# DeepGraphLearning/ULTRA

Measured on AMD Instinct MI355X. Metric: triples scored/sec (all-tail ranking) on FB15k237, higher is better.
Workload: dtype f32

## Files before the change

### ultra_amd/csrc/layer0_kernels.hpp

```cpp
#pragma once

#include <hip/hip_runtime.h>

#include <cstdint>

#include "layer0_update.hpp"
#include "rspmm_kernels.hpp"
#include "torch_math.hpp"

namespace ultra {

__global__ void __launch_bounds__(256) nbf_layer0_fill_kernel(const Layer0Params p) {
    __shared__ __attribute__((aligned(16))) float lds_slot[16 * 80];
    const int l16 = threadIdx.x & 15;
    const L0Vec vec = l0_load_vectors(p, l16);
    float c0[4];
#pragma unroll
    for (int e = 0; e < 4; ++e) c0[e] = vec.bias[e];
    l0_finish(c0, p, vec, lds_slot + (threadIdx.x >> 4) * 80, l16);
    const float4 v = make_float4(c0[0], c0[1], c0[2], c0[3]);
    if (p.out_sr == 64 && p.out_so == p.num_node * 64) {
        float4 *o4 = reinterpret_cast<float4 *>(p.out);
        const long long n16 = (long long)p.n_outer * p.num_node * 16;
        for (long long i = (long long)blockIdx.x * blockDim.x + threadIdx.x; i < n16; i += (long long)gridDim.x * blockDim.x) o4[i] = v;
        return;
    }
    const long long total = (long long)p.n_outer * p.num_node;
    const long long g0 = ((long long)blockIdx.x * blockDim.x + threadIdx.x) >> 4, ng = ((long long)gridDim.x * blockDim.x) >> 4;
    for (long long r = g0; r < total; r += ng) {
        const long long b = r / p.num_node, n = r - b * p.num_node;
        *reinterpret_cast<float4 *>(p.out + b * p.out_so + n * p.out_sr + 4 * l16) = v;
    }
}

__global__ void __launch_bounds__(1024) nbf_layer0_rows_kernel(const Layer0Params p) {
    __shared__ __attribute__((aligned(16))) float lds_wt[128 * 64];
    __shared__ __attribute__((aligned(16))) float lds_vec[64 * 80];
    const int outer = blockIdx.y;
    const int l16 = threadIdx.x & 15;
    const int grp = blockIdx.x * (blockDim.x >> 4) + (threadIdx.x >> 4);
    const int ngrp = gridDim.x * (blockDim.x >> 4);
    long long s = p.src[outer];
    s = s < 0 ? 0 : (s >= p.num_node ? p.num_node - 1 : s);
    const int k0 = p.trow_ptr[s], k1 = p.trow_ptr[s + 1];
    if (blockIdx.x > 0 && k0 + (int)blockIdx.x * (int)(blockDim.x >> 4) >= k1) return;
    const L0Vec vec = l0_load_vectors(p, l16);
    float qv[4];
#pragma unroll
    for (int e = 0; e < 4; ++e) qv[e] = p.q ? p.q[(long long)outer * 64 + 4 * l16 + e] : 1.f;
    {
        const int f = threadIdx.x & 63;
#pragma unroll
        for (int kc = 4 * (threadIdx.x >> 6); kc < 128; kc += 4 * (blockDim.x >> 6)) {
            const float4 wv = *reinterpret_cast<const float4 *>(p.weight + f * 128 + kc);
            lds_wt[(kc + 0) * 64 + f] = wv.x;
            lds_wt[(kc + 1) * 64 + f] = wv.y;
            lds_wt[(kc + 2) * 64 + f] = wv.z;
            lds_wt[(kc + 3) * 64 + f] = wv.w;
        }
    }
    __syncthreads();
    const float *relb = reinterpret_cast<const float *>(p.rel.ptr) + outer * p.rel.stride_outer;
    float *outb = p.out + outer * p.out_so;
    float *slot = lds_vec + (threadIdx.x >> 4) * 80;

    const auto update_row = [&](const float (&agg)[4], bool is_src, long long row) {
        float y[4] = {0.f, 0.f, 0.f, 0.f};
        if (is_src) {
            *reinterpret_cast<float4 *>(slot + 4 * l16) = make_float4(qv[0], qv[1], qv[2], qv[3]);
#pragma unroll
            for (int k4 = 0; k4 < 16; ++k4) {
                const float4 x4 = *reinterpret_cast<const float4 *>(slot + 4 * k4);
                const float xs[4] = {x4.x, x4.y, x4.z, x4.w};
#pragma unroll
                for (int e = 0; e < 4; ++e) {
                    const float4 wv = *reinterpret_cast<const float4 *>(lds_wt + (4 * k4 + e) * 64 + 4 * l16);
                    y[0] = __builtin_fmaf(xs[e], wv.x, y[0]);
                    y[1] = __builtin_fmaf(xs[e], wv.y, y[1]);
                    y[2] = __builtin_fmaf(xs[e], wv.z, y[2]);
                    y[3] = __builtin_fmaf(xs[e], wv.w, y[3]);
                }
            }
        }
        *reinterpret_cast<float4 *>(slot + 4 * l16) = make_float4(agg[0], agg[1], agg[2], agg[3]);
#pragma unroll
        for (int k4 = 0; k4 < 16; ++k4) {
            const float4 a4 = *reinterpret_cast<const float4 *>(slot + 4 * k4);
            const float as[4] = {a4.x, a4.y, a4.z, a4.w};
#pragma unroll
            for (int e = 0; e < 4; ++e) {
                const float4 wv = *reinterpret_cast<const float4 *>(lds_wt + (64 + 4 * k4 + e) * 64 + 4 * l16);
                y[0] = __builtin_fmaf(as[e], wv.x, y[0]);
                y[1] = __builtin_fmaf(as[e], wv.y, y[1]);
                y[2] = __builtin_fmaf(as[e], wv.z, y[2]);
                y[3] = __builtin_fmaf(as[e], wv.w, y[3]);
            }
        }
#pragma unroll
        for (int e = 0; e < 4; ++e) y[e] += vec.bias[e];
        l0_finish(y, p, vec, slot, l16);
        if (is_src && (p.flags & L0_RESIDUAL)) {
#pragma unroll
            for (int e = 0; e < 4; ++e) y[e] += qv[e];
        }
        *reinterpret_cast<float4 *>(outb + row * p.out_sr + 4 * l16) = make_float4(y[0], y[1], y[2], y[3]);
    };

    for (int k = k0 + grp; k < k1; k += ngrp) {
        const int last = k1 - 1;
        const int prev = p.tcol[k > k0 ? k - 1 : k0];
        int tc[4];
#pragma unroll
        for (int u = 0; u < 4; ++u) tc[u] = p.tcol[min(k + u, last)];
        const int target = tc[0];
        if (k > k0 && prev == target) continue;
        int kend = k + 1;
        if (kend < k1 && tc[1] == target) ++kend;
        if (kend == k + 2 && kend < k1 && tc[2] == target) ++kend;
        if (kend == k + 3 && kend < k1 && tc[3] == target) ++kend;
        if (kend == k + 4)
            while (kend < k1 && p.tcol[kend] == target) ++kend;
        const bool is_src = target == (int)s;
        const bool use_max = (p.flags & L0_MAX) != 0;
        const float init = (use_max && is_src && !(p.self_loop[s] & 2)) ? -3.402823466e+38f : 0.f;
        float agg[4] = {init, init, init, init};
        for (int kb = k; kb < kend; kb += 4) {
            float4 rv[4];
            float wv[4];
#pragma unroll
            for (int u = 0; u < 4; ++u) {
                const int kk = min(kb + u, kend - 1);
                const int ty = p.ttype[kk];
                rv[u] = *reinterpret_cast<const float4 *>(relb + (long long)ty * p.rel.stride_row + 4 * l16);
                wv[u] = p.w ? p.w[p.tperm[kk]] : 1.f;
            }
#pragma unroll
            for (int u = 0; u < 4; ++u) {
                if (kb + u < kend) {
                    const float r4[4] = {rv[u].x, rv[u].y, rv[u].z, rv[u].w};
#pragma unroll
                    for (int e = 0; e < 4; ++e) {
                        float m = r4[e] * qv[e];
                        if (p.w) m = wv[u] * m;
                        agg[e] = use_max ? fmaxf(agg[e], m) : agg[e] + m;
                    }
                }
            }
        }
        if (is_src) {
#pragma unroll
            for (int e = 0; e < 4; ++e) agg[e] = use_max ? fmaxf(agg[e], qv[e]) : agg[e] + qv[e];
        }
        update_row(agg, is_src, target);
    }
    if (grp == 0 && !(p.self_loop[s] & 1)) {
        float a0[4];
#pragma unroll
        for (int e = 0; e < 4; ++e) a0[e] = ((p.flags & L0_MAX) && (p.self_loop[s] & 2)) ? fmaxf(qv[e], 0.f) : qv[e];
        update_row(a0, true, s);
    }
}

}
```

### ultra_amd/csrc/layer0_update.hpp

```cpp
#pragma once

#include <hip/hip_runtime.h>

#include <cstdint>

#include "rspmm_kernels.hpp"
#include "torch_math.hpp"

namespace ultra {

enum { L0_LN = 1, L0_RELU = 2, L0_RESIDUAL = 4, L0_MAX = 8, L0_ONLY_FILL = 16, L0_SKIP_FILL = 32 };

struct Layer0Params {
    const int32_t *trow_ptr;
    const int32_t *tcol;
    const int32_t *ttype;
    const int32_t *tperm;
    const uint8_t *self_loop;
    const float *w;
    const int64_t *src;
    const float *q;
    MatArg rel;
    const float *weight;
    const float *bias, *ln_w, *ln_b;
    float *out;
    long long out_so, out_sr;
    long long num_node;
    int32_t n_outer;
    float eps;
    int32_t flags;
};

struct L0Vec {
    float bias[4], ln_w[4], ln_b[4];
};

__device__ __forceinline__ L0Vec l0_load_vectors(const Layer0Params &p, int l16) {
    L0Vec v;
#pragma unroll
    for (int e = 0; e < 4; ++e) {
        v.bias[e] = p.bias ? p.bias[4 * l16 + e] : 0.f;
        v.ln_w[e] = (p.flags & L0_LN) ? p.ln_w[4 * l16 + e] : 1.f;
        v.ln_b[e] = (p.flags & L0_LN) ? p.ln_b[4 * l16 + e] : 0.f;
    }
    return v;
}

__device__ __forceinline__ void l0_finish(float (&y)[4], const Layer0Params &p, const L0Vec &vec, float *slot, const int l16) {
    if (p.flags & L0_LN) {
        *reinterpret_cast<float4 *>(slot + 4 * l16) = make_float4(y[0], y[1], y[2], y[3]);
        float xv[8];
#pragma unroll
        for (int j = 0; j < 8; ++j) xv[j] = slot[8 * j + (l16 & 7)];
        const Moments w = welford8(xv);
        if (l16 < 8) {
            slot[64 + 2 * l16] = w.m1;
            slot[64 + 2 * l16 + 1] = w.m2;
        }
        Moments all[8];
#pragma unroll
        for (int i = 0; i < 8; ++i) all[i] = Moments{slot[64 + 2 * i], slot[64 + 2 * i + 1]};
        float mean, rstd;
        merge8(all, p.eps, mean, rstd);
#pragma unroll
        for (int e = 0; e < 4; ++e) y[e] = ln_apply(y[e], mean, rstd, vec.ln_w[e], vec.ln_b[e]);
    }
    if (p.flags & L0_RELU) {
#pragma unroll
        for (int e = 0; e < 4; ++e) y[e] = fmaxf(y[e], 0.f);
    }
}

}
```

### ultra_amd/csrc/rspmm_api.hip

```cpp
#include <hip/hip_runtime.h>

#include <cstdio>
#include <cstring>
#include <functional>
#include <string>
#include <vector>

#include "device_scope.hpp"
#include "layer0_kernels.hpp"
#include "rspmm_bwd_kernels.hpp"
#include "rspmm_kernels.hpp"
#include "rspmm_order_kernels.hpp"
#include "rspmm_rows_kernels.hpp"
#include "rows_bwd_kernels.hpp"

namespace ultra {

#define ULTRA_EXTERN_VARIANT(T_, VEC_, MODE_) \
    template <>                               \
    hipError_t launch_fwd_variant<T_, VEC_, MODE_>(int, int, const FwdParams &, int, int, size_t, hipStream_t);
ULTRA_EXTERN_VARIANT(float, 4, 0)
ULTRA_EXTERN_VARIANT(float, 1, 0)
ULTRA_EXTERN_VARIANT(float, 4, 1)
ULTRA_EXTERN_VARIANT(float, 4, 2)
// ... 596 lines not shown
    const int64_t step = dtype == ULTRA_F32 ? 4 : 2;
    bool vec4 = (row_len % 4 == 0) && mat_vec_ok(out, step);
    if (mul != BIN_RHS) vec4 = vec4 && mat_vec_ok(rel, step);
    if (mul != BIN_LHS) vec4 = vec4 && mat_vec_ok(x, step);
    if (bnd) vec4 = vec4 && mat_vec_ok(bnd, step);
    if (rot) vec4 = vec4 && (row_len % 8 == 0);
    const int VEC = vec4 ? 4 : 1;
    const int SPAN = 16 * VEC;
    const bool rot_far = rot && !(VEC == 4 && row_len == SPAN);

    if ((p->flags & ULTRA_PLAN_TYPE_RUNS) && !(p->flags & ULTRA_PLAN_EXACT_ORDER)) {
        if (!(sum == ULTRA_SUM_ADD && mul == BIN_MUL)) {
            set_error("a ULTRA_PLAN_TYPE_RUNS plan serves add_mul only (distributivity)");
            return ULTRA_ERR_UNSUPPORTED;
        }
        mul = BIN_MUL_TYPED;
    }
    const auto slice_bytes = [&](const ultra_mat *m, int64_t rows) { return (uint64_t)rows * (uint64_t)m->stride_row * esz; };
    if ((mul != BIN_LHS && slice_bytes(x, p->num_in) >= (1ull << 32)) ||
        (mul != BIN_RHS && slice_bytes(rel, p->num_rel) >= (1ull << 32))) {
        set_error("rspmm: an operand slice (rows * stride_row) exceeds 4 GiB; use the batch-major layout");
        return ULTRA_ERR_UNSUPPORTED;
    }
    FwdParams fp = fwd_params(p, mul, w, rel, x, bnd, out, SPAN, (int64_t)esz, call);

    const size_t ring_bytes = p->n_chain > 0 ? (size_t)2 * CHAIN_SLOTS * 64 * esz : 0;
    if ((p->flags & ULTRA_PLAN_EXACT_ORDER) && !rot && VEC == 4 && general_walk() == 0 && p->num_in < (1 << 24) &&
        p->num_rel < (1 << 24) && (mul == BIN_LHS || x->stride_row * (int64_t)esz < (1 << 24)) &&
        (mul == BIN_RHS || rel->stride_row * (int64_t)esz < (1 << 24)) && ring_bytes <= di.lds_optin)
        return forward_order(p, sum, mul, dtype, w, x, bnd, out, stream, call, fp, di, ring_bytes, point_fill);
    if (call.upd) {
        set_error("ultra_rspmm_forward_update: this call is not served by the reference-order kernels");
        return ULTRA_ERR_UNSUPPORTED;
    }
    if (call.w_samples) {
        set_error("ultra_rspmm_forward_masked_samples: this call is not served by the reference-order kernels (row length, "
                  "alignment or tuning)");
        return ULTRA_ERR_UNSUPPORTED;
    }
    if (point_fill) {
        set_error("a point boundary under min / max: this call is not served by the reference-order kernels (row length, "
                  "alignment or tuning); pass the boundary as a tensor");
        return ULTRA_ERR_UNSUPPORTED;
    }
    return forward_walk(p, sum, mul, dtype, w, bnd, out, stream, call, fp, di, VEC, rot_far);
}

static int ensure_backward_plans(ultra_plan *p) {
    if (p->tplan && p->rplan) return ULTRA_OK;
    if ((int64_t)p->h_row.size() != p->num_edge) return invalid("plan was built without its edge list; backward unavailable");
    ultra_plan_opts o;
    std::memset(&o, 0, sizeof(o));
    o.seg_len = p->seg_len;
    o.g_max = p->g_max;
    o.flags = p->flags & ~ULTRA_PLAN_EXACT_ORDER;
    if (!p->tplan) {
        p->tplan = build_plan(p->h_col.data(), p->h_row.data(), p->h_type.data(), p->num_edge, p->num_in, p->num_out,
                              p->num_rel, &o, false);
        p->tplan->pinned = p->pinned;
    }
    if (!p->rplan) {
        p->rplan = build_plan(p->h_type.data(), p->h_col.data(), p->h_row.data(), p->num_edge, p->num_rel, p->num_in,
                              p->num_out, &o, false);
        p->rplan->pinned = p->pinned;
    }
    return ULTRA_OK;
}

template <typename Launch>
static int backward_gather(ultra_plan *p, int dtype, const void *w, const EdgeParams &ep, const ultra_mat *xgrad,
                           const ultra_mat *rgrad, int32_t spans_per_outer, int fix_vec, const char *what, hipStream_t stream,
                           const Launch &launch) {
    const size_t esz = dtype == ULTRA_F32 ? 4 : 8;
    int rc;
    if ((rc = ensure_backward_plans(p))) return rc;
    for (int which = 0; which < 2; ++which) {
        ultra_plan *q = which == 0 ? p->tplan : p->rplan;
        const ultra_mat *dst = which == 0 ? xgrad : rgrad;
        if ((rc = upload_plan(q))) return rc;
        if (q->n_slot > 0 &&
            (rc = ensure_scratch(&q->d.partial, &q->d.partial_bytes, (size_t)q->n_slot * ep.n_outer * ep.row_len * esz, q)))
            return rc;
        GatherBwdParams gp;
        std::memset(&gp, 0, sizeof(gp));
        gp.items = q->d.items;
        gp.n_item = (int32_t)q->items.size();
        gp.col = q->d.col, gp.type = q->d.type, gp.perm = q->d.perm;
        gp.w = w;
        gp.rel = ep.rel, gp.x = ep.x, gp.out = ep.out, gp.og = ep.og;
        gp.grad = dst->ptr, gp.grad_so = dst->stride_outer, gp.grad_sr = dst->stride_row;
        gp.partial = q->d.partial;
        gp.n_outer = ep.n_outer, gp.row_len = ep.row_len;
        gp.spans_per_outer = spans_per_outer;
        gp.n_span = gp.spans_per_outer * gp.n_outer;
        const int grid = 2048;
        gp.smod = std::min<int32_t>(gp.n_span, grid);
        gp.nparts = grid / gp.smod;
        const hipError_t e = launch(which == 1, gp, grid);
        if (e != hipSuccess) return hip_fail(e, what);
        if ((rc = launch_fixup(q, dst, 0, dtype, fix_vec, stream))) return rc;
    }
    return ULTRA_OK;
}

static int backward_impl(ultra_plan *p, int sum, int mul, int dtype, const void *w, const ultra_mat *rel,
                         const ultra_mat *x, const ultra_mat *outm, const ultra_mat *og, void *wgrad,
                         const ultra_mat *rgrad, const ultra_mat *xgrad, hipStream_t stream, const ultra_mat *xbase = nullptr) {
    if (!p) return invalid("plan is NULL");
    if (xbase && (sum != ULTRA_SUM_ADD || !xgrad)) return invalid("input_grad_base is served under sum == add, with an input_grad");
    (void)hipGetLastError();
    if (p->flags & ULTRA_PLAN_DENSE) return invalid("a ULTRA_PLAN_DENSE plan has no backward; use the (row, col) plan");
    if (sum < 0 || sum > 2 || mul < 0 || mul > ULTRA_MUL_ROTATE) return invalid("unknown sum/mul code");
    const bool rot = mul == ULTRA_MUL_ROTATE;
    if (dtype != ULTRA_F32 && dtype != ULTRA_F64) return invalid("dtype must be ULTRA_F32 or ULTRA_F64");
    if (!og || !og->ptr) return invalid("output_grad is NULL");
    const int64_t n_outer = og->n_outer, row_len = og->row_len;
    if (n_outer <= 0 || row_len <= 0) return invalid("output_grad: empty n_outer / row_len");
    if (rot && (row_len & 1)) return invalid("rotate: row_len must be even (a row is real half | imaginary half)");
    int rc;
    if ((rc = check_mat(rel, "relation", p->num_rel, n_outer, row_len))) return rc;
    if ((rc = check_mat(x, "input", p->num_in, n_outer, row_len))) return rc;
    if ((rc = check_mat(outm, "output", p->num_out, n_outer, row_len))) return rc;
    if ((rc = check_mat(og, "output_grad", p->num_out, n_outer, row_len))) return rc;
    if ((rc = check_mat(rgrad, "relation_grad", p->num_rel, n_outer, row_len))) return rc;
    if (!xgrad && sum != ULTRA_SUM_ADD) return invalid("input_grad may be NULL under sum == add only");
    if (xgrad && (rc = check_mat(xgrad, "input_grad", p->num_in, n_outer, row_len))) return rc;
    if (xbase && (rc = check_mat(xbase, "input_grad_base", p->num_in, n_outer, row_len))) return rc;
    if ((rc = upload_plan(p))) return rc;

    const int64_t step = dtype == ULTRA_F32 ? 4 : 2;
    const bool vec4 = (row_len % 4 == 0) && mat_vec_ok(rel, step) && mat_vec_ok(x, step) && mat_vec_ok(outm, step) &&
                      mat_vec_ok(og, step) && mat_vec_ok(rgrad, step) && (!xgrad || mat_vec_ok(xgrad, step));

    EdgeParams ep;
    std::memset(&ep, 0, sizeof(ep));
    ep.erow = p->d.erow;
    ep.col = p->d.col;
    ep.type = p->d.type;
    ep.perm = p->d.perm;
    ep.w = w;
    ep.num_edge = p->num_edge;
    ep.num_out = (int32_t)p->num_out;
    ep.rel = MatArg{rel->ptr, rel->stride_outer, rel->stride_row};
    ep.x = MatArg{x->ptr, x->stride_outer, x->stride_row};
    ep.out = MatArg{outm->ptr, outm->stride_outer, outm->stride_row};
    ep.og = MatArg{og->ptr, og->stride_outer, og->stride_row};
    ep.rgrad = rgrad->ptr;
    ep.rgrad_so = rgrad->stride_outer;
    ep.rgrad_sr = rgrad->stride_row;
    ep.xgrad = xgrad ? xgrad->ptr : nullptr;
    ep.xgrad_so = xgrad ? xgrad->stride_outer : 0;
    ep.xgrad_sr = xgrad ? xgrad->stride_row : 0;
    ep.wgrad = wgrad;
    ep.n_outer = (int32_t)n_outer;
    ep.row_len = (int32_t)row_len;

    if (sum == ULTRA_SUM_ADD) {
        if ((rc = ensure_backward_plans(p))) return rc;
        if (xgrad && (rc = forward_impl(p->tplan, ULTRA_SUM_ADD, rot ? BIN_ROT_CREL : mul == ULTRA_MUL_MUL ? BIN_MUL : BIN_RHS, dtype,
                                        w, rel, og, xbase, xgrad, stream)))
            return rc;
        if ((rc = forward_impl(p->rplan, ULTRA_SUM_ADD, rot ? BIN_ROT_CX : mul == ULTRA_MUL_MUL ? BIN_MUL : BIN_LHS, dtype, w, og, x,
                               nullptr, rgrad, stream)))
            return rc;
        if (!wgrad || p->num_edge <= 0) return ULTRA_OK;
        if (rot) return launch_rot_edge_kernel(dtype, sum, false, ep, stream);
        return launch_edge_kernel(dtype, vec4 ? 4 : 1, sum, mul, false, ep, stream);
    }
    if (rot && p->num_edge > 0) {
        const bool fix4 = (row_len % 4 == 0) && mat_vec_ok(rgrad, step) && mat_vec_ok(xgrad, step);
        const auto launch = [&](bool rel_grad, const GatherBwdParams &gp, int grid) {
            return dtype == ULTRA_F32 ? launch_rot_gather_bwd_t<float>(sum, rel_grad, gp, grid, stream)
                                      : launch_rot_gather_bwd_t<double>(sum, rel_grad, gp, grid, stream);
        };
        if ((rc = backward_gather(p, dtype, w, ep, xgrad, rgrad, (int32_t)((row_len / 2 + 15) / 16), fix4 ? 4 : 1,
                                  "rspmm_rot_minmax_bwd_gather_kernel launch", stream, launch)))
            return rc;
        return wgrad ? launch_rot_edge_kernel(dtype, sum, false, ep, stream) : ULTRA_OK;
    }
    if (vec4 && row_len % 4 == 0 && p->num_edge > 0) {
        const auto launch = [&](bool rel_grad, const GatherBwdParams &gp, int grid) {
            return dtype == ULTRA_F32 ? launch_gather_bwd_t<float>(sum, mul, rel_grad, gp, grid, stream)
                                      : launch_gather_bwd_t<double>(sum, mul, rel_grad, gp, grid, stream);
        };
        if ((rc = backward_gather(p, dtype, w, ep, xgrad, rgrad, (int32_t)((row_len + 63) / 64), 4,
                                  "rspmm_minmax_bwd_gather_kernel launch", stream, launch)))
            return rc;
        return wgrad ? launch_edge_kernel(dtype, 4, sum, mul, false, ep, stream) : ULTRA_OK;
    }
    if ((rc = launch_fill_zero(dtype, rgrad, p->num_rel, stream))) return rc;
    if ((rc = launch_fill_zero(dtype, xgrad, p->num_in, stream))) return rc;
    if (p->num_edge > 0 && !rot) return launch_edge_kernel(dtype, vec4 ? 4 : 1, sum, mul, true, ep, stream);
    return ULTRA_OK;
}

static int forward_onehot_impl(ultra_plan *p, int dtype, const void *w, const ultra_mat *rel, const ultra_mat *x,
                               const int64_t *src_rows, const ultra_mat *bnd, const ultra_mat *out, hipStream_t stream) {
    if (!p) return invalid("plan is NULL");
    (void)hipGetLastError();
    if (dtype != ULTRA_F32 && dtype != ULTRA_F64) return invalid("dtype must be ULTRA_F32 or ULTRA_F64");
    if (!out || !out->ptr || !src_rows) return invalid("output / src_rows is NULL");
    if (p->flags & (ULTRA_PLAN_TYPE_RUNS | ULTRA_PLAN_DENSE)) return invalid("use the (row, col) plan for the one-hot path");
    const int64_t n_outer = out->n_outer, row_len = out->row_len;
    int rc;
    if ((rc = check_mat(out, "output", p->num_out, n_outer, row_len))) return rc;
    if ((rc = check_mat(rel, "relation", p->num_rel, n_outer, row_len))) return rc;
    if ((rc = check_mat(x, "input", p->num_in, n_outer, row_len))) return rc;
    if (bnd && (rc = check_mat(bnd, "boundary", p->num_out, n_outer, row_len))) return rc;
    if (p->num_out != p->num_in) return invalid("one-hot path needs a square graph (source rows are output rows)");
    if ((rc = ensure_backward_plans(p))) return rc;
    if ((rc = upload_plan(p->tplan))) return rc;
    const size_t esz = dtype == ULTRA_F32 ? 4 : 8;
    if (out->stride_row == row_len && (n_outer == 1 || out->stride_outer == out->n_row * row_len) && out->n_row == p->num_out &&
        aligned16(out->ptr) && ((size_t)n_outer * p->num_out * row_len * esz) % 16 == 0) {
        const long long n16 = (long long)((size_t)n_outer * p->num_out * row_len * esz / 16);
        hipLaunchKernelGGL(zero16_kernel, dim3(1024), dim3(256), 0, stream, reinterpret_cast<float4 *>(out->ptr), n16);
        HIP_TRY(hipGetLastError());
    } else if ((rc = launch_fill_zero(dtype, out, p->num_out, stream))) {
        return rc;
    }
    const int64_t step = dtype == ULTRA_F32 ? 4 : 2;
    const bool vec4 = (row_len % 4 == 0) && mat_vec_ok(out, step) && mat_vec_ok(rel, step) && mat_vec_ok(x, step);
    OneHotParams op;
    std::memset(&op, 0, sizeof(op));
    op.trow_ptr = p->tplan->d.row_ptr;
    op.tcol = p->tplan->d.col;
    op.ttype = p->tplan->d.type;
    op.tperm = p->tplan->d.perm;
    op.w = w;
    op.src = src_rows;
    op.rel = MatArg{rel->ptr, rel->stride_outer, rel->stride_row};
    op.x = MatArg{x->ptr, x->stride_outer, x->stride_row};
    if (bnd) op.bnd = MatArg{bnd->ptr, bnd->stride_outer, bnd->stride_row};
    op.out = out->ptr;
    op.out_so = out->stride_outer;
    op.out_sr = out->stride_row;
    op.n_outer = (int32_t)n_outer;
    op.row_len = (int32_t)row_len;
    op.has_bnd = bnd ? 1 : 0;
    const dim3 grid(64, (unsigned)n_outer), block(256);
    if (dtype == ULTRA_F32) {
        if (vec4) hipLaunchKernelGGL((rspmm_onehot_kernel<float, 4>), grid, block, 0, stream, op);
        else hipLaunchKernelGGL((rspmm_onehot_kernel<float, 1>), grid, block, 0, stream, op);
    } else {
        if (vec4) hipLaunchKernelGGL((rspmm_onehot_kernel<double, 4>), grid, block, 0, stream, op);
        else hipLaunchKernelGGL((rspmm_onehot_kernel<double, 1>), grid, block, 0, stream, op);
    }
    HIP_TRY(hipGetLastError());
    return ULTRA_OK;
}

static int layer0_impl(ultra_plan *p, const void *w, const ultra_mat *rel, const int64_t *src_rows, const void *src_vals,
                       const void *weight, const void *bias, const void *ln_w, const void *ln_b, float eps, int flags,
                       const ultra_mat *out, hipStream_t stream) {
    if (!p) return invalid("plan is NULL");
    (void)hipGetLastError();
    const bool only_fill = (flags & L0_ONLY_FILL) != 0;
    if (flags & ~(L0_LN | L0_RELU | L0_RESIDUAL | L0_MAX | L0_ONLY_FILL | L0_SKIP_FILL))
        return invalid("ultra_nbf_layer0: unknown flag bits " + std::to_string(flags & ~(L0_LN | L0_RELU | L0_RESIDUAL | L0_MAX | L0_ONLY_FILL | L0_SKIP_FILL)));
    if (only_fill && (flags & L0_SKIP_FILL)) return invalid("ultra_nbf_layer0: ULTRA_LAYER0_ONLY_FILL excludes ULTRA_LAYER0_SKIP_FILL");
    if (!out || !out->ptr || (!only_fill && (!src_rows || !weight))) return invalid("ultra_nbf_layer0: NULL operand");
    if ((flags & L0_LN) && (!ln_w || !ln_b)) return invalid("ultra_nbf_layer0: LayerNorm needs its weight and bias");
    if (p->flags & (ULTRA_PLAN_TYPE_RUNS | ULTRA_PLAN_DENSE)) return invalid("use the (row, col) plan for the layer-0 path");
    if (out->row_len != 64) {
        set_error("ultra_nbf_layer0: only hidden dim 64 is built (the ULTRA checkpoints' shape)");
        return ULTRA_ERR_UNSUPPORTED;
    }
    const int64_t n_outer = out->n_outer;
    int rc;
    if ((rc = check_mat(out, "output", p->num_out, n_outer, 64))) return rc;
    if (!only_fill && (rc = check_mat(rel, "relation", p->num_rel, n_outer, 64))) return rc;
    if (p->num_out != p->num_in) return invalid("layer-0 path needs a square graph (source rows are output rows)");
    if (!mat_vec_ok(out, 4) || (!only_fill && (!mat_vec_ok(rel, 4) || !aligned16(weight) || (src_vals && !aligned16(src_vals)))))
        return invalid("ultra_nbf_layer0: operands must be 16-byte aligned with strides that are multiples of 4");
    if (n_outer == 0 || p->num_out == 0) return ULTRA_OK;
    Layer0Params lp;
    std::memset(&lp, 0, sizeof(lp));
    if (!only_fill) {
        if ((rc = ensure_backward_plans(p))) return rc;
        if ((rc = upload_plan(p->tplan))) return rc;
        if ((rc = upload_plan(p))) return rc;
        if (!p->d.self_loop) return invalid("plan was built without its edge list; layer-0 path unavailable");
        lp.trow_ptr = p->tplan->d.row_ptr;
        lp.tcol = p->tplan->d.col;
        lp.ttype = p->tplan->d.type;
        lp.tperm = p->tplan->d.perm;
        lp.self_loop = p->d.self_loop;
        lp.rel = MatArg{rel->ptr, rel->stride_outer, rel->stride_row};
    }
    lp.w = static_cast<const float *>(w);
    lp.src = src_rows;
    lp.q = static_cast<const float *>(src_vals);
    lp.weight = static_cast<const float *>(weight);
    lp.bias = static_cast<const float *>(bias);
    lp.ln_w = static_cast<const float *>(ln_w);
    lp.ln_b = static_cast<const float *>(ln_b);
    lp.out = static_cast<float *>(out->ptr);
    lp.out_so = out->stride_outer;
    lp.out_sr = out->stride_row;
    lp.num_node = p->num_out;
    lp.n_outer = (int32_t)n_outer;
    lp.eps = eps;
    lp.flags = flags;
    const long long rows = (long long)n_outer * p->num_out;
    const int fill_blocks = (int)std::min<long long>((rows + 15) / 16, 1024);
    if (!(flags & L0_SKIP_FILL)) {
        hipLaunchKernelGGL(nbf_layer0_fill_kernel, dim3(fill_blocks), dim3(256), 0, stream, lp);
        HIP_TRY(hipGetLastError());
    }
    if (!only_fill) {
        ultra_plan *tp = p->tplan;
        if (tp->max_row_len < 0) {
            int32_t m = 0;
            for (size_t r = 0; r + 1 < tp->row_ptr.size(); ++r) m = std::max(m, tp->row_ptr[r + 1] - tp->row_ptr[r]);
            tp->max_row_len = m;
        }
        const unsigned l0_blocks = (unsigned)std::min(std::max((tp->max_row_len + 63) / 64, 32), 256);
        hipLaunchKernelGGL(nbf_layer0_rows_kernel, dim3(l0_blocks, (unsigned)n_outer), dim3(1024), 0, stream, lp);
        HIP_TRY(hipGetLastError());
    }
    return ULTRA_OK;
}

static int internal_mul(int32_t *mul) {
    if (*mul < 0 || *mul > ULTRA_MUL_ROTATE) return invalid("unknown mul code");
    if (*mul == ULTRA_MUL_ROTATE) *mul = BIN_ROT;
    return ULTRA_OK;
}

static int forward_update(ultra_plan *plan, int sum, int mul, const ultra_mat *relation, const ultra_mat *input,
                          const ultra_mat *point_values, const ultra_mat *aggregate, const void *weight, const void *bias,
                          const void *ln_weight, const void *ln_bias, float eps, int flags, const ultra_mat *output,
                          hipStream_t stream, FwdCall call) {
    if (mul < 0 || mul > 1) return invalid("unknown mul code");
    if ((call.bnd_rows == nullptr) != (point_values == nullptr)) return invalid("ultra_rspmm_forward_update: half a point boundary");
    if (!weight || !output || !output->ptr || !aggregate || !aggregate->ptr || ((flags & CONV_LN) && (!ln_weight || !ln_bias)))
        return invalid("ultra_rspmm_forward_update: NULL operand");
    if (flags & ~(CONV_LN | CONV_RELU | CONV_RESIDUAL | CONV_DBG_NO_MATRIX | CONV_DBG_NO_UPDATE | CONV_DBG_LOSE_ARRIVAL))
        return invalid("ultra_rspmm_forward_update: unknown flag");
    if (!plan) return invalid("plan is NULL");
    if (output->row_len != 64 || output->n_outer != aggregate->n_outer || output->n_row != aggregate->n_row ||
        output->stride_row < 64 || (output->stride_row % 4) != 0 || (output->stride_outer % 4) != 0 ||
        (reinterpret_cast<uintptr_t>(output->ptr) & 15) || output->ptr == aggregate->ptr || (input && output->ptr == input->ptr))
        return invalid("ultra_rspmm_forward_update: output must be a 16-byte aligned (n_outer, num_node, 64) tensor of its own");
    OrderParams::Update u;
    std::memset(&u, 0, sizeof(u));
    u.weight = (const float *)weight, u.bias = (const float *)bias;
    u.ln_w = (const float *)ln_weight, u.ln_b = (const float *)ln_bias;
    u.out = (float *)output->ptr;
    u.out_stride_outer = output->stride_outer, u.out_stride_row = output->stride_row;
    u.eps = eps, u.flags = flags;
    call.upd = &u;
    return forward_impl(plan, sum, mul, ULTRA_F32, nullptr, relation, input, point_values, aggregate, stream, call);
}

static ultra_mat dense2d(const void *ptr, int64_t rows, int64_t dim) {
    ultra_mat m;
    m.ptr = const_cast<void *>(ptr);
    m.n_outer = 1;
    m.stride_outer = 0;
    m.n_row = rows;
    m.stride_row = dim;
    m.row_len = dim;
    return m;
}

static int stateless_plan(ultra_plan **plan, const int64_t *ei_dev, const int64_t *et_dev, int64_t E, int64_t N,
                          int64_t R, hipStream_t stream) {
    *plan = nullptr;
    if (E < 0 || N < 0 || R < 0) return invalid("negative size");
    std::vector<int64_t> ei((size_t)2 * E), et((size_t)E);
    HIP_TRY(hipStreamSynchronize(stream));
    if (E > 0) {
        HIP_TRY(hipMemcpy(ei.data(), ei_dev, sizeof(int64_t) * 2 * E, hipMemcpyDeviceToHost));
        HIP_TRY(hipMemcpy(et.data(), et_dev, sizeof(int64_t) * E, hipMemcpyDeviceToHost));
        int64_t maxc = 0;
        for (int64_t e = 0; e < E; ++e) maxc = std::max(maxc, ei[(size_t)(E + e)]);
        for (int64_t e = 1; e < E; ++e) {
            const int64_t k0 = ei[(size_t)e - 1] * (maxc + 1) + ei[(size_t)(E + e - 1)];
            const int64_t k1 = ei[(size_t)e] * (maxc + 1) + ei[(size_t)(E + e)];
            if (k1 < k0) {
                set_error("Expect sorted `edge_index`");
                return ULTRA_ERR_UNSORTED;
            }
        }
    }
    ultra_plan_opts opts;
    std::memset(&opts, 0, sizeof(opts));
    opts.flags = ULTRA_PLAN_EXACT_ORDER;
    return ultra_plan_create(plan, ei.data(), et.data(), E, N, N, R, &opts);
}

}

using namespace ultra;

extern "C" {

int32_t ultra_device_count(void) {
    int n = 0;
    if (hipGetDeviceCount(&n) != hipSuccess) return 0;
    return n;
}

int32_t ultra_plan_upload(ultra_plan *plan) {
    if (!plan) return invalid("plan is NULL");
    return upload_plan(plan);
}

int32_t ultra_plan_pin(ultra_plan *plan, int32_t delta) {
    if (!plan) return invalid("plan is NULL");
    const auto bump = [&](ultra_plan *q) { q->pinned = std::max<int32_t>(0, q->pinned + delta); };
    bump(plan);
    if (plan->tplan) bump(plan->tplan);
    if (plan->rplan) bump(plan->rplan);
    return ULTRA_OK;
}

int32_t ultra_plan_destroy(ultra_plan *plan) {
    if (!plan) return ULTRA_OK;
    if (plan->tplan) ultra_plan_destroy(plan->tplan);
    if (plan->rplan) ultra_plan_destroy(plan->rplan);
    free_device(plan);
    delete plan;
    return ULTRA_OK;
}

int32_t ultra_rspmm_weight_epoch(int64_t epoch) {
    g_w_epoch = epoch;
    return ULTRA_OK;
}

int32_t ultra_rspmm_forward(ultra_plan *plan, int32_t sum, int32_t mul, int32_t dtype, const void *edge_weight_dev,
                            const ultra_mat *relation, const ultra_mat *input, const ultra_mat *boundary,
                            const ultra_mat *output, void *stream) {
    ULTRA_DEVICE_SCOPE(stream, output ? output->ptr : nullptr);
    WeightEpochScope weight_epoch_scope;
    if (int rc = internal_mul(&mul)) return rc;
    return forward_impl(plan, sum, mul, dtype, edge_weight_dev, relation, input, boundary, output,
                        reinterpret_cast<hipStream_t>(stream));
}

int32_t ultra_rspmm_forward_masked(ultra_plan *plan, int32_t sum, int32_t mul, int32_t dtype, const void *edge_keep_dev,
                                   const ultra_mat *relation, const ultra_mat *input, const ultra_mat *boundary,
                                   const ultra_mat *output, void *stream) {
    ULTRA_DEVICE_SCOPE(stream, output ? output->ptr : nullptr);
    WeightEpochScope weight_epoch_scope;
    if (int rc = internal_mul(&mul)) return rc;
    if (!edge_keep_dev) return invalid("ultra_rspmm_forward_masked: edge_keep is NULL");
    FwdCall call;
    call.keep_mode = 1;
    return forward_impl(plan, sum, mul, dtype, edge_keep_dev, relation, input, boundary, output,
                        reinterpret_cast<hipStream_t>(stream), call);
}

int32_t ultra_rspmm_forward_masked_samples(ultra_plan *plan, int32_t sum, int32_t mul, int32_t dtype, const void *edge_keep_dev,
                                           int64_t keep_stride, const ultra_mat *relation, const ultra_mat *input,
                                           const ultra_mat *boundary, const ultra_mat *output, void *stream) {
    if (!plan) return invalid("plan is NULL");
    if (keep_stride < plan->num_edge) return invalid("ultra_rspmm_forward_masked_samples: keep_stride < num_edge");
    if (!edge_keep_dev) return invalid("ultra_rspmm_forward_masked_samples: edge_keep is NULL");
    if (!output || !output->ptr) return invalid("output is NULL");
    if (output->n_outer == 0) return ULTRA_OK;
    if (keep_stride > INT32_MAX) {
        set_error("ultra_rspmm_forward_masked_samples: keep_stride beyond 2^31 - 1 elements");
        return ULTRA_ERR_UNSUPPORTED;
    }
    ULTRA_DEVICE_SCOPE(stream, output->ptr);
    WeightEpochScope weight_epoch_scope;
    if (int rc = internal_mul(&mul)) return rc;
    FwdCall call;
    call.keep_mode = 1;
    call.w_samples = true;
    call.w_stride_outer = keep_stride;
    return forward_impl(plan, sum, mul, dtype, edge_keep_dev, relation, input, boundary, output,
                        reinterpret_cast<hipStream_t>(stream), call);
}

int32_t ultra_rspmm_forward_point(ultra_plan *plan, int32_t sum, int32_t mul, int32_t dtype, const void *edge_weight_dev,
                                  const ultra_mat *relation, const ultra_mat *input, const int64_t *point_rows_dev,
                                  const ultra_mat *point_values, const ultra_mat *output, void *stream) {
    ULTRA_DEVICE_SCOPE(stream, output ? output->ptr : nullptr);
    WeightEpochScope weight_epoch_scope;
    if (int rc = internal_mul(&mul)) return rc;
    if (!point_rows_dev || !point_values) return invalid("ultra_rspmm_forward_point: NULL point boundary");
    return forward_impl(plan, sum, mul, dtype, edge_weight_dev, relation, input, point_values, output,
                        reinterpret_cast<hipStream_t>(stream), FwdCall{point_rows_dev});
}

int32_t ultra_rspmm_forward_update(ultra_plan *plan, int32_t sum, int32_t mul, const ultra_mat *relation, const ultra_mat *input,
                                   const int64_t *point_rows_dev, const ultra_mat *point_values, const ultra_mat *aggregate,
                                   const void *weight, const void *bias, const void *ln_weight, const void *ln_bias, float eps,
                                   int32_t flags, const ultra_mat *output, void *stream) {
    ULTRA_DEVICE_SCOPE(stream, output ? output->ptr : nullptr);
    return forward_update(plan, sum, mul, relation, input, point_values, aggregate, weight, bias, ln_weight, ln_bias, eps, flags,
                          output, reinterpret_cast<hipStream_t>(stream), FwdCall{point_rows_dev});
}

int32_t ultra_rspmm_forward_onehot(ultra_plan *plan, int32_t dtype, const void *edge_weight_dev,
                                   const ultra_mat *relation, const ultra_mat *input, const int64_t *src_rows_dev,
                                   const ultra_mat *boundary, const ultra_mat *output, void *stream) {
    ULTRA_DEVICE_SCOPE(stream, output ? output->ptr : nullptr);
    return forward_onehot_impl(plan, dtype, edge_weight_dev, relation, input, src_rows_dev, boundary, output,
                               reinterpret_cast<hipStream_t>(stream));
}

int32_t ultra_nbf_layer0(ultra_plan *plan, const void *edge_weight_dev, const ultra_mat *relation, const int64_t *src_rows_dev,
                         const void *src_values_dev, const void *weight, const void *bias, const void *ln_weight,
                         const void *ln_bias, float eps, int32_t flags, const ultra_mat *output, void *stream) {
    ULTRA_DEVICE_SCOPE(stream, output ? output->ptr : nullptr);
    return layer0_impl(plan, edge_weight_dev, relation, src_rows_dev, src_values_dev, weight, bias, ln_weight, ln_bias, eps,
                       flags, output, reinterpret_cast<hipStream_t>(stream));
}

int32_t ultra_nbf_dense_layer(ultra_plan *plan, const ultra_mat *relation, const ultra_mat *input, const ultra_mat *boundary,
                              const int64_t *point_rows_dev, const void *weight, const void *bias, const void *ln_weight,
                              const void *ln_bias, float eps, int32_t flags, const ultra_mat *output, void *stream) {
    ULTRA_DEVICE_SCOPE(stream, output ? output->ptr : nullptr);
    if (!plan) return invalid("plan is NULL");
    (void)hipGetLastError();
    if (!output || !output->ptr || !weight) return invalid("ultra_nbf_dense_layer: NULL operand");
    if ((flags & 1) && (!ln_weight || !ln_bias)) return invalid("ultra_nbf_dense_layer: LayerNorm needs its weight and bias");
    if (point_rows_dev && !boundary) return invalid("ultra_nbf_dense_layer: point rows without their values");
    const int64_t n_outer = output->n_outer;
    int rc;
    if ((rc = check_mat(output, "output", plan->num_out, n_outer, output->row_len))) return rc;
    if ((rc = check_mat(relation, "relation", plan->num_rel, n_outer, output->row_len))) return rc;
    if ((rc = check_mat(input, "input", plan->num_in, n_outer, output->row_len))) return rc;
    if (boundary && (rc = check_mat(boundary, "boundary", point_rows_dev ? 1 : plan->num_out, n_outer, output->row_len))) return rc;
    if (n_outer == 0 || plan->num_out == 0) return ULTRA_OK;
    if ((rc = upload_plan(plan))) return rc;
    if (flags & ULTRA_LAYER_REFERENCE_ORDER) {
        DevInfo di;
        if ((rc = device_info(&di))) return rc;
        const bool shared_chip = g_tuning.grid > 0 && g_tuning.grid < di.cu;
        return launch_dense_order_layer(plan, relation, input, boundary, point_rows_dev, weight, bias, ln_weight, ln_bias, eps,
                                        flags & 7, output, reinterpret_cast<hipStream_t>(stream), shared_chip);
    }
    return launch_dense_layer(plan, relation, input, boundary, point_rows_dev, weight, bias, ln_weight, ln_bias, eps, flags,
                              output, reinterpret_cast<hipStream_t>(stream));
}

static int check_adjacency(const char *name, const void *a_ex_dev, int64_t num_node) {
    if (!a_ex_dev) return invalid(std::string(name) + ": the adjacency is NULL");
    if (num_node <= 0 || num_node > ULTRA_DENSE_MAX_IN_ROW)
        return invalid(std::string(name) + ": num_node must lie in [1, " + std::to_string(ULTRA_DENSE_MAX_IN_ROW) + "], got " +
                       std::to_string((long long)num_node));
    return ULTRA_OK;
}

int32_t ultra_nbf_dense_layer_adjacency(const void *a_ex_dev, int64_t num_node, const ultra_mat *relation, const ultra_mat *input,
                                        const ultra_mat *boundary, const int64_t *point_rows_dev, const void *weight,
                                        const void *bias, const void *ln_weight, const void *ln_bias, float eps, int32_t flags,
                                        const ultra_mat *output, void *stream) {
    ULTRA_DEVICE_SCOPE(stream, output ? output->ptr : nullptr);
    (void)hipGetLastError();
    int rc;
    if ((rc = check_adjacency("ultra_nbf_dense_layer_adjacency", a_ex_dev, num_node))) return rc;
    if (!(flags & ULTRA_LAYER_REFERENCE_ORDER))
        return invalid("ultra_nbf_dense_layer_adjacency: served in the reference's order only (ULTRA_LAYER_REFERENCE_ORDER)");
    if (!output || !output->ptr || !weight) return invalid("ultra_nbf_dense_layer_adjacency: NULL operand");
    if ((flags & 1) && (!ln_weight || !ln_bias)) return invalid("ultra_nbf_dense_layer_adjacency: LayerNorm needs its weight and bias");
    if (point_rows_dev && !boundary) return invalid("ultra_nbf_dense_layer_adjacency: point rows without their values");
    const int64_t n_outer = output->n_outer;
    if ((rc = check_mat(output, "output", num_node, n_outer, output->row_len))) return rc;
    if ((rc = check_mat(relation, "relation", 4, n_outer, output->row_len))) return rc;
    if ((rc = check_mat(input, "input", num_node, n_outer, output->row_len))) return rc;
    if (boundary && (rc = check_mat(boundary, "boundary", point_rows_dev ? 1 : num_node, n_outer, output->row_len))) return rc;
    if (n_outer == 0) return ULTRA_OK;
    DevInfo di;
    if ((rc = device_info(&di))) return rc;
    const bool shared_chip = g_tuning.grid > 0 && g_tuning.grid < di.cu;
    return launch_dense_order_layer_adjacency(a_ex_dev, num_node, relation, input, boundary, point_rows_dev, weight, bias, ln_weight,
                                              ln_bias, eps, flags & 7, output, reinterpret_cast<hipStream_t>(stream), shared_chip);
}

int32_t ultra_nbf_dense_layer0_adjacency(const void *a_ex_dev, int64_t num_node, const ultra_mat *relation, const int64_t *src_rows_dev,
                                         const void *src_values_dev, const void *weight, const void *bias, const void *ln_weight,
                                         const void *ln_bias, float eps, int32_t flags, const ultra_mat *output, void *stream) {
    ULTRA_DEVICE_SCOPE(stream, output ? output->ptr : nullptr);
    (void)hipGetLastError();
    int rc;
    if ((rc = check_adjacency("ultra_nbf_dense_layer0_adjacency", a_ex_dev, num_node))) return rc;
    if (flags & ~(L0_LN | L0_RELU | L0_RESIDUAL | L0_MAX))
        return invalid("ultra_nbf_dense_layer0_adjacency: unknown flag bits " + std::to_string(flags & ~(L0_LN | L0_RELU | L0_RESIDUAL | L0_MAX)));
    if (!output || !output->ptr || !src_rows_dev || !weight) return invalid("ultra_nbf_dense_layer0_adjacency: NULL operand");
    if ((flags & L0_LN) && (!ln_weight || !ln_bias)) return invalid("ultra_nbf_dense_layer0_adjacency: LayerNorm needs its weight and bias");
    if (output->row_len != 64 || (flags & L0_MAX)) {
        set_error("ultra_nbf_dense_layer0_adjacency: the sum aggregate at hidden dim 64 (weight (64, 128)) in fp32 only");
        return ULTRA_ERR_UNSUPPORTED;
    }
    const int64_t n_outer = output->n_outer;
    if ((rc = check_mat(output, "output", num_node, n_outer, 64))) return rc;
    if ((rc = check_mat(relation, "relation", 4, n_outer, 64))) return rc;
    if (n_outer > 65535) return invalid("ultra_nbf_dense_layer0_adjacency: at most 65535 samples a launch");
    if (!mat_vec_ok(output, 4) || !mat_vec_ok(relation, 4) || !aligned16(weight) || (src_values_dev && !aligned16(src_values_dev)))
        return invalid("ultra_nbf_dense_layer0_adjacency: operands must be 16-byte aligned with strides that are multiples of 4");
    if (n_outer == 0) return ULTRA_OK;
    return launch_dense_layer0_adjacency(a_ex_dev, num_node, relation, src_rows_dev, src_values_dev, weight, bias, ln_weight, ln_bias,
                                         eps, flags, output, reinterpret_cast<hipStream_t>(stream));
}

int32_t ultra_rspmm_backward(ultra_plan *plan, int32_t sum, int32_t mul, int32_t dtype, const void *edge_weight_dev,
                             const ultra_mat *relation, const ultra_mat *input, const ultra_mat *output,
                             const ultra_mat *output_grad, void *weight_grad_dev, const ultra_mat *relation_grad,
                             const ultra_mat *input_grad, void *stream) {
// ... 495 lines not shown
```

Before: 213.9 million.

## Fuse layer-0 fill and special-row update into one sliced kernel

Replaces the separate fill kernel and rows kernel with a single kernel. Each block owns a slice of output nodes, marks which rows are touched by the source's edges in a shared bitmap, writes the constant fill only to untouched rows, and then computes the edge-aggregated rows for that slice. The goal is to avoid writing those rows twice, save a kernel launch, and spread the special-row work across slices. The cost is a per-block scan or binary search of the source row's edges, plus restaging the weight in LDS in every block that has special rows.

```diff
diff --git a/ultra_amd/csrc/layer0_kernels.hpp b/ultra_amd/csrc/layer0_kernels.hpp
--- a/ultra_amd/csrc/layer0_kernels.hpp
+++ b/ultra_amd/csrc/layer0_kernels.hpp
@@ -33,132 +33,238 @@
     }
 }
 
+template <int THREADS>
+__device__ __forceinline__ void l0_stage_weight(const float *weight, float *lds_wt) {
+    const int f = threadIdx.x & 63;
+#pragma unroll 4
+    for (int kc = 4 * (threadIdx.x >> 6); kc < 128; kc += 4 * (THREADS >> 6)) {
+        const float4 wv = *reinterpret_cast<const float4 *>(weight + f * 128 + kc);
+        lds_wt[(kc + 0) * 64 + f] = wv.x;
+        lds_wt[(kc + 1) * 64 + f] = wv.y;
+        lds_wt[(kc + 2) * 64 + f] = wv.z;
+        lds_wt[(kc + 3) * 64 + f] = wv.w;
+    }
+}
+
+struct L0Group {
+    int l16;
+    L0Vec vec;
+    float qv[4];
+    float *slot;
+    const float *lds_wt;
+    const float *relb;
+    float *outb;
+};
+
+__device__ __forceinline__ void l0_update_row(const Layer0Params &p, const L0Group &g, const float (&agg)[4], bool is_src, long long row) {
+    const int l16 = g.l16;
+    float y[4] = {0.f, 0.f, 0.f, 0.f};
+    if (is_src) {
+        *reinterpret_cast<float4 *>(g.slot + 4 * l16) = make_float4(g.qv[0], g.qv[1], g.qv[2], g.qv[3]);
+#pragma unroll
+        for (int k4 = 0; k4 < 16; ++k4) {
+            const float4 x4 = *reinterpret_cast<const float4 *>(g.slot + 4 * k4);
+            const float xs[4] = {x4.x, x4.y, x4.z, x4.w};
+#pragma unroll
+            for (int e = 0; e < 4; ++e) {
+                const float4 wv = *reinterpret_cast<const float4 *>(g.lds_wt + (4 * k4 + e) * 64 + 4 * l16);
+                y[0] = __builtin_fmaf(xs[e], wv.x, y[0]);
+                y[1] = __builtin_fmaf(xs[e], wv.y, y[1]);
+                y[2] = __builtin_fmaf(xs[e], wv.z, y[2]);
+                y[3] = __builtin_fmaf(xs[e], wv.w, y[3]);
+            }
+        }
+    }
+    *reinterpret_cast<float4 *>(g.slot + 4 * l16) = make_float4(agg[0], agg[1], agg[2], agg[3]);
+#pragma unroll
+    for (int k4 = 0; k4 < 16; ++k4) {
+        const float4 a4 = *reinterpret_cast<const float4 *>(g.slot + 4 * k4);
+        const float as[4] = {a4.x, a4.y, a4.z, a4.w};
+#pragma unroll
+        for (int e = 0; e < 4; ++e) {
+            const float4 wv = *reinterpret_cast<const float4 *>(g.lds_wt + (64 + 4 * k4 + e) * 64 + 4 * l16);
+            y[0] = __builtin_fmaf(as[e], wv.x, y[0]);
+            y[1] = __builtin_fmaf(as[e], wv.y, y[1]);
+            y[2] = __builtin_fmaf(as[e], wv.z, y[2]);
+            y[3] = __builtin_fmaf(as[e], wv.w, y[3]);
+        }
+    }
+#pragma unroll
+    for (int e = 0; e < 4; ++e) y[e] += g.vec.bias[e];
+    l0_finish(y, p, g.vec, g.slot, l16);
+    if (is_src && (p.flags & L0_RESIDUAL)) {
+#pragma unroll
+        for (int e = 0; e < 4; ++e) y[e] += g.qv[e];
+    }
+    *reinterpret_cast<float4 *>(g.outb + row * p.out_sr + 4 * l16) = make_float4(y[0], y[1], y[2], y[3]);
+}
+
+__device__ __forceinline__ void l0_special_rows(const Layer0Params &p, const L0Group &g, long long s, int ka, int kb, int grp, int ngrp,
+                                                bool own_src) {
+    const int l16 = g.l16;
+    for (int k = ka + grp; k < kb; k += ngrp) {
+        const int last = kb - 1;
+        const int prev = p.tcol[k > ka ? k - 1 : ka];
+        int tc[4];
+#pragma unroll
+        for (int u = 0; u < 4; ++u) tc[u] = p.tcol[min(k + u, last)];
+        const int target = tc[0];
+        if (k > ka && prev == target) continue;
+        int kend = k + 1;
+        if (kend < kb && tc[1] == target) ++kend;
+        if (kend == k + 2 && kend < kb && tc[2] == target) ++kend;
+        if (kend == k + 3 && kend < kb && tc[3] == target) ++kend;
+        if (kend == k + 4)
+            while (kend < kb && p.tcol[kend] == target) ++kend;
+        const bool is_src = target == (int)s;
+        const bool use_max = (p.flags & L0_MAX) != 0;
+        const float init = (use_max && is_src && !(p.self_loop[s] & 2)) ? -3.402823466e+38f : 0.f;
+        float agg[4] = {init, init, init, init};
+        for (int kq = k; kq < kend; kq += 4) {
+            float4 rv[4];
+            float wv[4];
+#pragma unroll
+            for (int u = 0; u < 4; ++u) {
+                const int kk = min(kq + u, kend - 1);
+                const int ty = p.ttype[kk];
+                rv[u] = *reinterpret_cast<const float4 *>(g.relb + (long long)ty * p.rel.stride_row + 4 * l16);
+                wv[u] = p.w ? p.w[p.tperm[kk]] : 1.f;
+            }
+#pragma unroll
+            for (int u = 0; u < 4; ++u) {
+                if (kq + u < kend) {
+                    const float r4[4] = {rv[u].x, rv[u].y, rv[u].z, rv[u].w};
+#pragma unroll
+                    for (int e = 0; e < 4; ++e) {
+                        float m = r4[e] * g.qv[e];
+                        if (p.w) m = wv[u] * m;
+                        agg[e] = use_max ? fmaxf(agg[e], m) : agg[e] + m;
+                    }
+                }
+            }
+        }
+        if (is_src) {
+#pragma unroll
+            for (int e = 0; e < 4; ++e) agg[e] = use_max ? fmaxf(agg[e], g.qv[e]) : agg[e] + g.qv[e];
+        }
+        l0_update_row(p, g, agg, is_src, target);
+    }
+    if (own_src && !(p.self_loop[s] & 1)) {
+        float a0[4];
+#pragma unroll
+        for (int e = 0; e < 4; ++e) a0[e] = ((p.flags & L0_MAX) && (p.self_loop[s] & 2)) ? fmaxf(g.qv[e], 0.f) : g.qv[e];
+        l0_update_row(p, g, a0, true, s);
+    }
+}
+
+__device__ __forceinline__ L0Group l0_group(const Layer0Params &p, int outer, const L0Vec &vec, float *slot, const float *lds_wt) {
+    L0Group g;
+    g.l16 = threadIdx.x & 15;
+    g.vec = vec;
+#pragma unroll
+    for (int e = 0; e < 4; ++e) g.qv[e] = p.q ? p.q[(long long)outer * 64 + 4 * g.l16 + e] : 1.f;
+    g.slot = slot;
+    g.lds_wt = lds_wt;
+    g.relb = reinterpret_cast<const float *>(p.rel.ptr) + outer * p.rel.stride_outer;
+    g.outb = p.out + outer * p.out_so;
+    return g;
+}
+
 __global__ void __launch_bounds__(1024) nbf_layer0_rows_kernel(const Layer0Params p) {
     __shared__ __attribute__((aligned(16))) float lds_wt[128 * 64];
     __shared__ __attribute__((aligned(16))) float lds_vec[64 * 80];
     const int outer = blockIdx.y;
-    const int l16 = threadIdx.x & 15;
     const int grp = blockIdx.x * (blockDim.x >> 4) + (threadIdx.x >> 4);
     const int ngrp = gridDim.x * (blockDim.x >> 4);
     long long s = p.src[outer];
     s = s < 0 ? 0 : (s >= p.num_node ? p.num_node - 1 : s);
     const int k0 = p.trow_ptr[s], k1 = p.trow_ptr[s + 1];
     if (blockIdx.x > 0 && k0 + (int)blockIdx.x * (int)(blockDim.x >> 4) >= k1) return;
+    const L0Group g = l0_group(p, outer, l0_load_vectors(p, threadIdx.x & 15), lds_vec + (threadIdx.x >> 4) * 80, lds_wt);
+    l0_stage_weight<1024>(p.weight, lds_wt);
+    __syncthreads();
+    l0_special_rows(p, g, s, k0, k1, grp, ngrp, grp == 0);
+}
+
+#ifndef ULTRA_L0_SLICE
+#define ULTRA_L0_SLICE 128
+#endif
+constexpr int L0_SLICE = ULTRA_L0_SLICE;
+constexpr int L0_SCAN_MAX = 2048;
+static_assert(L0_SLICE % 32 == 0 && L0_SLICE >= 32, "L0_SLICE: whole bitmap words");
+
+inline int l0_slice_len(long long num_node) {
+    const long long want = ((num_node + 31) / 32 + 15) / 16 * 16;
+    return (int)(want < 16 ? 16 : (want > L0_SLICE ? L0_SLICE : want));
+}
+
+__global__ void __launch_bounds__(512) nbf_layer0_kernel(const Layer0Params p) {
+    __shared__ __attribute__((aligned(16))) float lds_wt[128 * 64];
+    __shared__ __attribute__((aligned(16))) float lds_vec[16 * 80];
+    __shared__ unsigned special[L0_SLICE / 32];
+    __shared__ int span[2];
+    const int outer = blockIdx.y;
+    const int l16 = threadIdx.x & 15, grp = threadIdx.x >> 4;
+    const long long base = (long long)blockIdx.x * p.slice;
+    const int nrow = (int)min((long long)p.slice, p.num_node - base);
+    long long s = p.src[outer];
+    s = s < 0 ? 0 : (s >= p.num_node ? p.num_node - 1 : s);
+    const int k0 = p.trow_ptr[s], k1 = p.trow_ptr[s + 1];
+    if (threadIdx.x < L0_SLICE / 32) special[threadIdx.x] = 0u;
+    if (threadIdx.x == 0) {
+        span[0] = k1;
+        span[1] = k0;
+    }
+    const bool scan = k1 - k0 <= L0_SCAN_MAX;
+    int lo = k0, hi = k0;
+    if (!scan) {
+        const int t_lo = (int)base, t_hi = (int)base + nrow;
+        int n = k1 - k0;
+        while (n > 1) {
+            const int half = n >> 1;
+            const int a = p.tcol[lo + half - 1], b = p.tcol[hi + half - 1];
+            if (a < t_lo) lo += half;
+            if (b < t_hi) hi += half;
+            n -= half;
+        }
+        const int a = p.tcol[lo], b = p.tcol[hi];
+        lo += a < t_lo;
+        hi += b < t_hi;
+    }
+    const bool owns_src = s >= base && s < base + nrow;
     const L0Vec vec = l0_load_vectors(p, l16);
-    float qv[4];
-#pragma unroll
-    for (int e = 0; e < 4; ++e) qv[e] = p.q ? p.q[(long long)outer * 64 + 4 * l16 + e] : 1.f;
-    {
-        const int f = threadIdx.x & 63;
-#pragma unroll
-        for (int kc = 4 * (threadIdx.x >> 6); kc < 128; kc += 4 * (blockDim.x >> 6)) {
-            const float4 wv = *reinterpret_cast<const float4 *>(p.weight + f * 128 + kc);
-            lds_wt[(kc + 0) * 64 + f] = wv.x;
-            lds_wt[(kc + 1) * 64 + f] = wv.y;
-            lds_wt[(kc + 2) * 64 + f] = wv.z;
-            lds_wt[(kc + 3) * 64 + f] = wv.w;
-        }
-    }
-    __syncthreads();
-    const float *relb = reinterpret_cast<const float *>(p.rel.ptr) + outer * p.rel.stride_outer;
+    __syncthreads();
+    for (int k = (scan ? k0 : lo) + (int)threadIdx.x; k < (scan ? k1 : hi); k += 256) {
+        const int r = p.tcol[k] - (int)base;
+        if ((unsigned)r < (unsigned)nrow) {
+            atomicOr(&special[r >> 5], 1u << (r & 31));
+            if (scan) {
+                atomicMin(&span[0], k);
+                atomicMax(&span[1], k + 1);
+            }
+        }
+    }
+    if (owns_src && threadIdx.x == 0) atomicOr(&special[(int)(s - base) >> 5], 1u << ((int)(s - base) & 31));
+    float *slot = lds_vec + grp * 80;
+    float c0[4];
+#pragma unroll
+    for (int e = 0; e < 4; ++e) c0[e] = vec.bias[e];
+    l0_finish(c0, p, vec, slot, l16);
+    __syncthreads();
+    if (scan) {
+        lo = __builtin_amdgcn_readfirstlane(span[0]);
+        hi = __builtin_amdgcn_readfirstlane(span[1]);
+        if (hi <= lo) lo = hi = k0;
+    }
     float *outb = p.out + outer * p.out_so;
-    float *slot = lds_vec + (threadIdx.x >> 4) * 80;
-
-    const auto update_row = [&](const float (&agg)[4], bool is_src, long long row) {
-        float y[4] = {0.f, 0.f, 0.f, 0.f};
-        if (is_src) {
-            *reinterpret_cast<float4 *>(slot + 4 * l16) = make_float4(qv[0], qv[1], qv[2], qv[3]);
-#pragma unroll
-            for (int k4 = 0; k4 < 16; ++k4) {
-                const float4 x4 = *reinterpret_cast<const float4 *>(slot + 4 * k4);
-                const float xs[4] = {x4.x, x4.y, x4.z, x4.w};
-#pragma unroll
-                for (int e = 0; e < 4; ++e) {
-                    const float4 wv = *reinterpret_cast<const float4 *>(lds_wt + (4 * k4 + e) * 64 + 4 * l16);
-                    y[0] = __builtin_fmaf(xs[e], wv.x, y[0]);
-                    y[1] = __builtin_fmaf(xs[e], wv.y, y[1]);
-                    y[2] = __builtin_fmaf(xs[e], wv.z, y[2]);
-                    y[3] = __builtin_fmaf(xs[e], wv.w, y[3]);
-                }
-            }
-        }
-        *reinterpret_cast<float4 *>(slot + 4 * l16) = make_float4(agg[0], agg[1], agg[2], agg[3]);
-#pragma unroll
-        for (int k4 = 0; k4 < 16; ++k4) {
-            const float4 a4 = *reinterpret_cast<const float4 *>(slot + 4 * k4);
-            const float as[4] = {a4.x, a4.y, a4.z, a4.w};
-#pragma unroll
-            for (int e = 0; e < 4; ++e) {
-                const float4 wv = *reinterpret_cast<const float4 *>(lds_wt + (64 + 4 * k4 + e) * 64 + 4 * l16);
-                y[0] = __builtin_fmaf(as[e], wv.x, y[0]);
-                y[1] = __builtin_fmaf(as[e], wv.y, y[1]);
-                y[2] = __builtin_fmaf(as[e], wv.z, y[2]);
-                y[3] = __builtin_fmaf(as[e], wv.w, y[3]);
-            }
-        }
-#pragma unroll
-        for (int e = 0; e < 4; ++e) y[e] += vec.bias[e];
-        l0_finish(y, p, vec, slot, l16);
-        if (is_src && (p.flags & L0_RESIDUAL)) {
-#pragma unroll
-            for (int e = 0; e < 4; ++e) y[e] += qv[e];
-        }
-        *reinterpret_cast<float4 *>(outb + row * p.out_sr + 4 * l16) = make_float4(y[0], y[1], y[2], y[3]);
-    };
-
-    for (int k = k0 + grp; k < k1; k += ngrp) {
-        const int last = k1 - 1;
-        const int prev = p.tcol[k > k0 ? k - 1 : k0];
-        int tc[4];
-#pragma unroll
-        for (int u = 0; u < 4; ++u) tc[u] = p.tcol[min(k + u, last)];
-        const int target = tc[0];
-        if (k > k0 && prev == target) continue;
-        int kend = k + 1;
-        if (kend < k1 && tc[1] == target) ++kend;
-        if (kend == k + 2 && kend < k1 && tc[2] == target) ++kend;
-        if (kend == k + 3 && kend < k1 && tc[3] == target) ++kend;
-        if (kend == k + 4)
-            while (kend < k1 && p.tcol[kend] == target) ++kend;
-        const bool is_src = target == (int)s;
-        const bool use_max = (p.flags & L0_MAX) != 0;
-        const float init = (use_max && is_src && !(p.self_loop[s] & 2)) ? -3.402823466e+38f : 0.f;
-        float agg[4] = {init, init, init, init};
-        for (int kb = k; kb < kend; kb += 4) {
-            float4 rv[4];
-            float wv[4];
-#pragma unroll
-            for (int u = 0; u < 4; ++u) {
-                const int kk = min(kb + u, kend - 1);
-                const int ty = p.ttype[kk];
-                rv[u] = *reinterpret_cast<const float4 *>(relb + (long long)ty * p.rel.stride_row + 4 * l16);
-                wv[u] = p.w ? p.w[p.tperm[kk]] : 1.f;
-            }
-#pragma unroll
-            for (int u = 0; u < 4; ++u) {
-                if (kb + u < kend) {
-                    const float r4[4] = {rv[u].x, rv[u].y, rv[u].z, rv[u].w};
-#pragma unroll
-                    for (int e = 0; e < 4; ++e) {
-                        float m = r4[e] * qv[e];
-                        if (p.w) m = wv[u] * m;
-                        agg[e] = use_max ? fmaxf(agg[e], m) : agg[e] + m;
-                    }
-                }
-            }
-        }
-        if (is_src) {
-#pragma unroll
-            for (int e = 0; e < 4; ++e) agg[e] = use_max ? fmaxf(agg[e], qv[e]) : agg[e] + qv[e];
-        }
-        update_row(agg, is_src, target);
-    }
-    if (grp == 0 && !(p.self_loop[s] & 1)) {
-        float a0[4];
-#pragma unroll
-        for (int e = 0; e < 4; ++e) a0[e] = ((p.flags & L0_MAX) && (p.self_loop[s] & 2)) ? fmaxf(qv[e], 0.f) : qv[e];
-        update_row(a0, true, s);
-    }
-}
-
-}
+    const float4 v = make_float4(c0[0], c0[1], c0[2], c0[3]);
+    for (int r = grp; r < nrow; r += 16)
+        if (!((special[r >> 5] >> (r & 31)) & 1u)) *reinterpret_cast<float4 *>(outb + (base + r) * p.out_sr + 4 * l16) = v;
+    if (hi == lo && !owns_src) return;
+    const L0Group g = l0_group(p, outer, vec, slot, lds_wt);
+    l0_stage_weight<256>(p.weight, lds_wt);
+    __syncthreads();
+    l0_special_rows(p, g, s, lo, hi, grp, 16, grp == 0 && owns_src);
+}
+
+}
diff --git a/ultra_amd/csrc/layer0_update.hpp b/ultra_amd/csrc/layer0_update.hpp
--- a/ultra_amd/csrc/layer0_update.hpp
+++ b/ultra_amd/csrc/layer0_update.hpp
@@ -29,6 +29,7 @@
     int32_t n_outer;
     float eps;
     int32_t flags;
+    int32_t slice;
 };
 
 struct L0Vec {
diff --git a/ultra_amd/csrc/rspmm_api.hip b/ultra_amd/csrc/rspmm_api.hip
--- a/ultra_amd/csrc/rspmm_api.hip
+++ b/ultra_amd/csrc/rspmm_api.hip
@@ -922,6 +922,13 @@
     lp.n_outer = (int32_t)n_outer;
     lp.eps = eps;
     lp.flags = flags;
+    if (!(flags & (L0_ONLY_FILL | L0_SKIP_FILL))) {
+        lp.slice = l0_slice_len(p->num_out);
+        const unsigned slices = (unsigned)((p->num_out + lp.slice - 1) / lp.slice);
+        hipLaunchKernelGGL(nbf_layer0_kernel, dim3(slices, (unsigned)n_outer), dim3(256), 0, stream, lp);
+        HIP_TRY(hipGetLastError());
+        return ULTRA_OK;
+    }
     const long long rows = (long long)n_outer * p->num_out;
     const int fill_blocks = (int)std::min<long long>((rows + 15) / 16, 1024);
     if (!(flags & L0_SKIP_FILL)) {
```

Measured after the change: 215.0 million (median of 2 runs). No clear change (+0.5%).
